# k2kobayashi/crank

Hardware: AMD Instinct MI355X
Metric: train frames/sec (higher is better)
Workload: dtype bf16

## Files before the change

### crank_amd/csrc/vq_kernels.hip

```cpp
#include "common.h"
#include "switches.h"
void conv_prof_begin(int cls, double flops, hipStream_t s);
void conv_prof_end(int cls, hipStream_t s);
void conv_prof_bytes(int cls, double bytes);

#define VQ_FRAMES 128
#define VQ_FIX_SCALE 268435456.0f
#define VQ_FIX_INV 3.7252902984619140625e-9f

template <int D>
__global__ __launch_bounds__(512) void vq_forward_kernel(const float* __restrict__ x, int ldx,
                                                         const float* __restrict__ cb, int N, int K, int kchunk,
                                                         long long* __restrict__ idx_out, float* __restrict__ e_out,
                                                         int lde, float* __restrict__ qx_out, int ldq) {
  extern __shared__ __attribute__((aligned(16))) unsigned char smem[];
  float* cbs = reinterpret_cast<float*>(smem);
  float* w2s = cbs + (size_t)kchunk * D;
  float* red_d = w2s + kchunk;
  int* red_i = reinterpret_cast<int*>(red_d + 4 * VQ_FRAMES);
  const int tid = threadIdx.x, lane = tid & 63, wave = tid >> 6;
  const int fg = wave & 1, cg = wave >> 1;
  const int fl = fg * 64 + lane;
  const long n = (long)blockIdx.x * VQ_FRAMES + fl;
  const bool valid = n < N;
// ... 365 lines not shown
    const long nw = (long)blockIdx.x * VQM_FB + fg * 32;
#pragma unroll
    for (int g = tp * (8 / TP); g < (tp + 1) * (8 / TP); g++) {
      const int f = 4 * g + sub;
      const int bi = __shfl(besti, f, 64);
      const long nf = nw + f;
      if (nf < N) {
        const float4 e = *reinterpret_cast<const float4*>(cb + (size_t)bi * D + c4);
        if (e_out) *reinterpret_cast<float4*>(e_out + nf * (long)lde + c4) = e;
        float4 xv = make_float4(0.f, 0.f, 0.f, 0.f);
        if (qx_out || fz.xsum || fz.cpart) {
          xv = *reinterpret_cast<const float4*>(x + nf * (long)ldx + c4);
          if (fz.add) {
            const float4 av = *reinterpret_cast<const float4*>(fz.add + nf * (long)fz.ldadd + c4);
            xv.x += av.x; xv.y += av.y; xv.z += av.z; xv.w += av.w;
          }
          if (fz.xsum) *reinterpret_cast<float4*>(fz.xsum + nf * (long)fz.ldsum + c4) = xv;
        }
        if (fz.cpart && (!fz.mask || fz.mask[nf])) {
          const float d0 = xv.x - e.x, d1 = xv.y - e.y, d2 = xv.z - e.z, d3 = xv.w - e.w;
          csum += d0 * d0; csum += d1 * d1; csum += d2 * d2; csum += d3 * d3;
          ccnt += 4.f;
        }
        if (qx_out) {
          float4 o;
          o.x = xv.x + (e.x - xv.x);
          o.y = xv.y + (e.y - xv.y);
          o.z = xv.z + (e.z - xv.z);
          o.w = xv.w + (e.w - xv.w);
          *reinterpret_cast<float4*>(qx_out + nf * (long)ldq + c4) = o;
        }
      }
    }
  }
  if (fz.cpart) {
#pragma unroll
    for (int o = 32; o > 0; o >>= 1) { csum += __shfl_xor(csum, o, 64); ccnt += __shfl_xor(ccnt, o, 64); }
    if (lane == 0) { vq_red[wave] = csum; vq_red[4 * TP + wave] = ccnt; }
    __syncthreads();
    if (tid == 0) {
      float a = vq_red[0], c = vq_red[4 * TP];
#pragma unroll
      for (int w = 1; w < 4 * TP; w++) { a += vq_red[w]; c += vq_red[4 * TP + w]; }
      fz.cpart[2 * blockIdx.x] = a; fz.cpart[2 * blockIdx.x + 1] = c;
    }
  }
  VQ_T(2)
}

typedef _Float16 vq_h8 __attribute__((ext_vector_type(8)));
typedef float vq_f32x2 __attribute__((ext_vector_type(2)));
typedef _Float16 vq_h4 __attribute__((ext_vector_type(4)));
#define VQH_KEY_EPS 1.6e-5f
#ifndef VQH_KEY_ABS
#define VQH_KEY_ABS 1.2e-38f
#endif
#define VQH_WS 68

__device__ unsigned long long vq_f16_flag_counts[3];
extern "C" int crk_debug_vq_flags(unsigned long long* host_out3, int reset) {
  if (hipMemcpyFromSymbol(host_out3, HIP_SYMBOL(vq_f16_flag_counts), 3 * sizeof(unsigned long long)) != hipSuccess) return 2;
  if (reset) {
    const unsigned long long z[3] = {0, 0, 0};
    if (hipMemcpyToSymbol(HIP_SYMBOL(vq_f16_flag_counts), z, sizeof(z)) != hipSuccess) return 2;
  }
  return 0;
}

__device__ __forceinline__ float vq_min_raw(float a, float b) {
  float r;
  asm("v_min_f32 %0, %1, %2" : "=v"(r) : "v"(a), "v"(b));
  return r;
}
struct VqTop3 { float m1, m2, m3; int i1, i2; };
__device__ __forceinline__ void vq_top3_insert(VqTop3& t, float v, int k) {
  const bool c1 = v < t.m1 || (v == t.m1 && k < t.i1);
  const bool c2 = v < t.m2 || (v == t.m2 && k < t.i2);
  t.m3 = c2 ? t.m2 : fminf(t.m3, v);
  t.i2 = c1 ? t.i1 : (c2 ? k : t.i2);
  t.m2 = c1 ? t.m1 : (c2 ? v : t.m2);
  t.i1 = c1 ? k : t.i1;
  t.m1 = c1 ? v : t.m1;
}
__device__ __forceinline__ void vq_top3_merge(VqTop3& t, float b1, float b2, float b3, int j1, int j2) {
  vq_top3_insert(t, b1, j1);
  vq_top3_insert(t, b2, j2);
  t.m3 = fminf(t.m3, b3);
}
__device__ __forceinline__ float vq_pow2(int e) { return __builtin_bit_cast(float, (unsigned)(e + 127) << 23); }
__device__ __forceinline__ int vq_expo(float v) { return (int)((__builtin_bit_cast(unsigned, v) >> 23) & 0xffu) - 127; }

#define VQ_PAD_W2 1.0e37f
__device__ __forceinline__ void vq_code_stats(const float* wrow, int k, int K, float& w2o, float& uswo, float& swso, float& wmxo) {
  float w2 = 0.f, am = 0.f;
#pragma unroll
  for (int q = 0; q < 16; q++) {
    const vq_f32x4 e = *reinterpret_cast<const vq_f32x4*>(wrow + 4 * q);
#pragma unroll
    for (int j = 0; j < 4; j++) { w2 = vq_sq_acc(w2, e[j]); am = fmaxf(am, fabsf(e[j])); }
  }
  w2o = k < K ? w2 : VQ_PAD_W2;
  const int er = 10 - vq_expo(am);
  const bool ok = am == 0.f || (w2 < INFINITY && er >= -60 && er <= 60);
  const int ewk = (ok && am > 0.f) ? er : 0;
  uswo = -2.f * vq_pow2(-ewk);
  swso = vq_pow2(ewk);
  wmxo = k < K ? (ok ? (w2 == w2 ? w2 : INFINITY) : INFINITY) : 0.f;
}
__device__ __forceinline__ void vq_plane_piece(vq_f32x4 pv, float sw, int k, int c, unsigned char* wh, unsigned char* wlo) {
  const int ct = k >> 5, i = k & 31, kc = c >> 2, h = (c & 3) >> 1;
  vq_h4 hi, lo;
#pragma unroll
  for (int jj = 0; jj < 4; jj++) {
    const float v = pv[jj] * sw;
    hi[jj] = (_Float16)v;
    lo[jj] = (_Float16)(v - (float)hi[jj]);
  }
  const size_t off = ((((size_t)ct * 4 + kc) * 64 + i + 32 * h) * 8 + 4 * (c & 1)) * 2;
  *reinterpret_cast<vq_h4*>(wh + off) = hi;
  *reinterpret_cast<vq_h4*>(wlo + off) = lo;
}
struct VqImgQ { const float* cb; unsigned char* img; int K; };
struct VqImgM { VqImgQ q[4]; };
__global__ __launch_bounds__(256) void vq_image_kernel(const VqImgM m) {
  __shared__ float wimg[32 * VQH_WS];
  __shared__ float sw_s[32];
  const VqImgQ e = m.q[blockIdx.y];
  const int K = e.K, KT = ((K + 63) >> 6) * 2, ct = blockIdx.x, tid = threadIdx.x;
  if (ct >= KT) return;
  vq_f32x4 pv[2];
#pragma unroll
  for (int j = 0; j < 2; j++) {
    const int pi = tid + 256 * j, k = ct * 32 + (pi >> 4);
    pv[j] = k < K ? *reinterpret_cast<const vq_f32x4*>(e.cb + (size_t)k * 64 + 4 * (pi & 15)) : vq_f32x4{0.f, 0.f, 0.f, 0.f};
    *reinterpret_cast<vq_f32x4*>(wimg + (size_t)(pi >> 4) * VQH_WS + 4 * (pi & 15)) = pv[j];
  }
  __syncthreads();
  float* tabs = reinterpret_cast<float*>(e.img + (size_t)KT * 8192);
  if (tid < 32) {
    const int k = ct * 32 + tid;
    float w2, us, sw, wm;
    vq_code_stats(wimg + (size_t)tid * VQH_WS, k, K, w2, us, sw, wm);
    tabs[k] = w2; tabs[KT * 32 + k] = us; tabs[2 * KT * 32 + k] = sw; tabs[3 * KT * 32 + k] = wm;
    sw_s[tid] = sw;
  }
  __syncthreads();
#pragma unroll
  for (int j = 0; j < 2; j++) {
    const int pi = tid + 256 * j;
    vq_plane_piece(pv[j], sw_s[pi >> 4], ct * 32 + (pi >> 4), pi & 15, e.img, e.img + (size_t)KT * 4096);
  }
}

template <int TP>
__global__ __launch_bounds__(256 * TP, 1) void vq_forward_f16_kernel(const float* __restrict__ x, int ldx,
                                                                     const float* __restrict__ cb, int N, int K,
                                                                     long long* __restrict__ idx_out, float* __restrict__ e_out,
                                                                     int lde, float* __restrict__ qx_out, int ldq, const VqFuse fz) {
  constexpr int D = 64, NT = 256 * TP;
  __shared__ float vq_red[8 * TP];
  __shared__ float vq_wmax[4 * TP];
  __shared__ float vq_m[TP][3][VQM_FB];
  __shared__ int vq_i[TP][2][VQM_FB];
  __shared__ float vq_xrow[4 * TP][D];
  extern __shared__ __attribute__((aligned(16))) unsigned char smem[];
  const int KT = ((K + 63) >> 6) * 2;
  unsigned char* wh = smem;
  unsigned char* wlo = smem + (size_t)KT * 4096;
  float* wimg = reinterpret_cast<float*>(smem);
  float* w2s = reinterpret_cast<float*>(smem + (size_t)KT * 32 * VQH_WS * 4);
  float* usw = w2s + KT * 32;
  float* sws = usw + KT * 32;
  const int tid = threadIdx.x, lane = tid & 63, l31 = lane & 31, half = lane >> 5;
  const int wave = __builtin_amdgcn_readfirstlane(tid >> 6), fg = wave & 3, tp = wave >> 2;
#ifdef VQ_PROF
  const unsigned long long vq_t0_ = __builtin_readcyclecounter();
#endif

  const long n = (long)blockIdx.x * VQM_FB + fg * 32 + l31;
  const bool valid = n < N;
  vq_f32x4 row[16];
  float w2max;
  if (fz.img) {
    constexpr int NPI = 16 / TP * 2;
    const vq_f32x4* src = reinterpret_cast<const vq_f32x4*>(fz.img);
    const float* tabs = reinterpret_cast<const float*>(fz.img + (size_t)KT * 8192);
    float* xt = reinterpret_cast<float*>(smem);
    constexpr int NXP = VQM_FB * 16 / NT;
    vq_f32x4 xv[NXP], av[NXP];
#pragma unroll
    for (int i = 0; i < NXP; i++) {
      const int pidx = tid + NT * i, f = pidx >> 4, c = pidx & 15;
      const long nf = (long)blockIdx.x * VQM_FB + f;
      xv[i] = nf < N ? *reinterpret_cast<const vq_f32x4*>(x + nf * (long)ldx + 4 * c) : vq_f32x4{0.f, 0.f, 0.f, 0.f};
      av[i] = (fz.add && nf < N) ? *reinterpret_cast<const vq_f32x4*>(fz.add + nf * (long)fz.ldadd + 4 * c) : vq_f32x4{0.f, 0.f, 0.f, 0.f};
    }
    vq_f32x4 pc[NPI];
#pragma unroll
    for (int j = 0; j < NPI; j++) { const int i = tid + NT * j; pc[j] = i < KT * 512 ? src[i] : vq_f32x4{0.f, 0.f, 0.f, 0.f}; }
    float tb[3];
#pragma unroll
    for (int j = 0; j < 3; j++) { const int i = tid + NT * j; tb[j] = i < 3 * KT * 32 ? tabs[i] : 0.f; }
    constexpr int NWM = (16 * 32 + NT - 1) / NT;
    float wm[NWM];
#pragma unroll
    for (int j = 0; j < NWM; j++) { const int k = tid + NT * j; wm[j] = k < KT * 32 ? tabs[3 * KT * 32 + k] : 0.f; }
#pragma unroll
    for (int i = 0; i < NXP; i++) {
      const int pidx = tid + NT * i;
      if (fz.add) xv[i] += av[i];
      if (fz.xsum_early) {
        const long nf = (long)blockIdx.x * VQM_FB + (pidx >> 4);
        if (nf < N) *reinterpret_cast<vq_f32x4*>(fz.xsum + nf * (long)fz.ldsum + 4 * (pidx & 15)) = xv[i];
      }
      *reinterpret_cast<vq_f32x4*>(xt + (size_t)(pidx >> 4) * VQH_WS + 4 * (pidx & 15)) = xv[i];
    }
    __syncthreads();
    {
      const float* xr = xt + (size_t)(fg * 32 + l31) * VQH_WS;
#pragma unroll
      for (int q = 0; q < 16; q++) row[q] = *reinterpret_cast<const vq_f32x4*>(xr + 4 * q);
    }
    __syncthreads();
    float wmx = 0.f;
#pragma unroll
    for (int j = 0; j < NWM; j++) wmx = fmaxf(wmx, wm[j]);
#pragma unroll
    for (int j = 0; j < NPI; j++) { const int i = tid + NT * j; if (i < KT * 512) reinterpret_cast<vq_f32x4*>(wh)[i] = pc[j]; }
#pragma unroll
    for (int j = 0; j < 3; j++) { const int i = tid + NT * j; if (i < 3 * KT * 32) w2s[i] = tb[j]; }
    for (int i = 3 * NT + tid; i < 3 * KT * 32; i += NT) w2s[i] = tabs[i];
#pragma unroll
    for (int o = 32; o > 0; o >>= 1) wmx = fmaxf(wmx, __shfl_xor(wmx, o, 64));
    if (lane == 0) vq_wmax[wave] = wmx;
    __syncthreads();
    w2max = vq_wmax[0];
#pragma unroll
    for (int w = 1; w < 4 * TP; w++) w2max = fmaxf(w2max, vq_wmax[w]);
  } else {
  {
    const float* xp = x + (valid ? n : 0) * (long)ldx;
#pragma unroll
    for (int q = 0; q < 16; q++) row[q] = *reinterpret_cast<const vq_f32x4*>(xp + 4 * q);
    if (fz.add) {
      const float* ap = fz.add + (valid ? n : 0) * (long)fz.ldadd;
#pragma unroll
      for (int q = 0; q < 16; q++) row[q] += *reinterpret_cast<const vq_f32x4*>(ap + 4 * q);
    }
  }
  constexpr int NPV = 16 / TP * 2;
  vq_f32x4 pv[NPV];
#pragma unroll
  for (int j = 0; j < NPV; j++) {
    const int pi = tid + NT * j, k = pi >> 4;
    pv[j] = (pi < KT * 32 * 16 && k < K) ? *reinterpret_cast<const vq_f32x4*>(cb + (size_t)pi * 4) : vq_f32x4{0.f, 0.f, 0.f, 0.f};
  }
#pragma unroll
  for (int j = 0; j < NPV; j++) {
    const int pi = tid + NT * j, k = pi >> 4, c = pi & 15;
    if (pi < KT * 32 * 16) *reinterpret_cast<vq_f32x4*>(wimg + (size_t)k * VQH_WS + 4 * c) = pv[j];
  }
  __syncthreads();
  float wmx = 0.f;
  for (int k = tid; k < KT * 32; k += NT) {
    float wm;
    vq_code_stats(wimg + (size_t)k * VQH_WS, k, K, w2s[k], usw[k], sws[k], wm);
    wmx = fmaxf(wmx, wm);
  }
#pragma unroll
  for (int o = 32; o > 0; o >>= 1) wmx = fmaxf(wmx, __shfl_xor(wmx, o, 64));
  if (lane == 0) vq_wmax[wave] = wmx;
  __syncthreads();
  w2max = vq_wmax[0];
#pragma unroll
  for (int w = 1; w < 4 * TP; w++) w2max = fmaxf(w2max, vq_wmax[w]);
  {
    float swk[NPV];
#pragma unroll
    for (int j = 0; j < NPV; j++) { const int pi = tid + NT * j; swk[j] = pi < KT * 32 * 16 ? sws[pi >> 4] : 1.f; }
#pragma unroll
    for (int j = 0; j < NPV; j++) {
      const int pi = tid + NT * j;
      if (pi < KT * 32 * 16) vq_plane_piece(pv[j], swk[j], pi >> 4, pi & 15, wh, wlo);
    }
  }
  }
  const bool w_ok = w2max < INFINITY;
  float x2 = 0.f, xmx = 0.f;
#pragma unroll
  for (int q = 0; q < 16; q++) {
#pragma unroll
    for (int j = 0; j < 4; j++) { x2 = vq_sq_acc(x2, row[q][j]); xmx = fmaxf(xmx, fabsf(row[q][j])); }
  }
  const int ex_raw = 10 - vq_expo(xmx);
  const bool x_ok = x2 < INFINITY && (xmx == 0.f || (ex_raw >= -60 && ex_raw <= 60));
  const int ex = (x_ok && xmx > 0.f) ? ex_raw : 0;
  vq_h8 xh[4], xl[4];
  {
    const float sx = vq_pow2(ex);
#pragma unroll
    for (int kc = 0; kc < 4; kc++)
#pragma unroll
      for (int j = 0; j < 8; j++) {
        const int d = 16 * kc + 8 * half + j;
        const float v0 = row[(16 * kc + j) >> 2][(16 * kc + j) & 3], v1 = row[(16 * kc + 8 + j) >> 2][(16 * kc + 8 + j) & 3];
        const float v = (half ? v1 : v0) * sx;
        (void)d;
        const _Float16 hi = (_Float16)v;
        xh[kc][j] = hi;
        xl[kc][j] = (_Float16)(v - (float)hi);
      }
  }
  const float sxinv = vq_pow2(-ex);
  __syncthreads();
  VQ_T(0)

  VqTop3 t;
  t.m1 = t.m2 = t.m3 = INFINITY;
  t.i1 = t.i2 = 0x7fffffff;
  const unsigned char* whl = wh + lane * 16;
  const unsigned char* wll = wlo + lane * 16;
#define VQH_TILE(aA, aB, ct, hc, lc, hn, ln)                                                                   \
  {                                                                                                            \
    _Pragma("unroll") for (int r = 0; r < 16; r++) { aA[r] = 0.f; aB[r] = 0.f; }                               \
    const size_t to_ = (size_t)((ct) + TP < KT ? (ct) + TP : (ct)) * 4096;                                     \
    _Pragma("unroll") for (int kc = 0; kc < 4; kc++) {                                                         \
      hn[kc] = *reinterpret_cast<const vq_h8*>(whl + to_ + kc * 1024);                                         \
      ln[kc] = *reinterpret_cast<const vq_h8*>(wll + to_ + kc * 1024);                                         \
    }                                                                                                          \
    _Pragma("unroll") for (int kc = 0; kc < 4; kc++) {                                                         \
      aA = __builtin_amdgcn_mfma_f32_32x32x16_f16(hc[kc], xh[kc], aA, 0, 0, 0);                                \
      aB = __builtin_amdgcn_mfma_f32_32x32x16_f16(lc[kc], xh[kc], aB, 0, 0, 0);                                \
      aB = __builtin_amdgcn_mfma_f32_32x32x16_f16(hc[kc], xl[kc], aB, 0, 0, 0);                                \
    }                                                                                                          \
  }
#define VQH_PICK(aA, aB, ct, tord) { const unsigned tagb_ = (unsigned)(tord) << 4; VQH_PICK_(aA, aB, ct) }
#define VQH_PICK_(aA, aB, ct)                                                                                  \
  _Pragma("unroll") for (int q = 0; q < 4; q++) {                                                              \
    const vq_f32x4 w2q = *reinterpret_cast<const vq_f32x4*>(w2s + (ct) * 32 + 8 * q + 4 * half);               \
    const vq_f32x4 usq = *reinterpret_cast<const vq_f32x4*>(usw + (ct) * 32 + 8 * q + 4 * half) * sxinv;       \
    _Pragma("unroll") for (int j2 = 0; j2 < 2; j2++) {                                                         \
      const vq_f32x2 acc = vq_f32x2{aA[4 * q + 2 * j2], aA[4 * q + 2 * j2 + 1]} +                              \
                           vq_f32x2{aB[4 * q + 2 * j2], aB[4 * q + 2 * j2 + 1]};                               \
      const vq_f32x2 v2 = __builtin_elementwise_fma(acc, vq_f32x2{usq[2 * j2], usq[2 * j2 + 1]},               \
                                                    vq_f32x2{w2q[2 * j2], w2q[2 * j2 + 1]});                   \
      const float vs_[2] = {v2.x, v2.y};      \
      _Pragma("unroll") for (int jj = 0; jj < 2; jj++) {                                                       \
        unsigned tag = tagb_ | (unsigned)(4 * q + 2 * j2 + jj);                                                \
        asm volatile("" : "+s"(tag));      \
        const float key = __builtin_bit_cast(float, (__builtin_bit_cast(unsigned, vs_[jj]) & keymask) | tag);  \
        t.m3 = __builtin_amdgcn_fmed3f(key, t.m2, t.m3);                                                       \
        t.m2 = __builtin_amdgcn_fmed3f(key, t.m1, t.m2);                                                       \
        t.m1 = vq_min_raw(key, t.m1);                                                                          \
      }                                                                                                        \
    }                                                                                                          \
  }
#define VQH_PAIR(nA, nB, ctn, hc, lc, hn, ln, pA, pB, ctp, tordp)                                              \
  VQH_TILE(nA, nB, ctn, hc, lc, hn, ln)                                                                        \
  VQH_PICK(pA, pB, ctp, tordp)                                                                                 \
  __builtin_amdgcn_sched_barrier(0);
  unsigned keymask = ~0x7fu;
  asm volatile("" : "+v"(keymask));
  f32x16 a0A, a0B, a1A, a1B;
  vq_h8 hA[4], lA[4], hB[4], lB[4];
#pragma unroll
  for (int kc = 0; kc < 4; kc++) {
    hA[kc] = *reinterpret_cast<const vq_h8*>(whl + (size_t)tp * 4096 + kc * 1024);
    lA[kc] = *reinterpret_cast<const vq_h8*>(wll + (size_t)tp * 4096 + kc * 1024);
  }
  VQH_TILE(a0A, a0B, tp, hA, lA, hB, lB)
  __builtin_amdgcn_sched_barrier(0);
  int tord = 0;
  for (int ct = tp; ct < KT - 2 * TP; ct += 2 * TP, tord += 2) {
    VQH_PAIR(a1A, a1B, ct + TP, hB, lB, hA, lA, a0A, a0B, ct, tord)
    VQH_PAIR(a0A, a0B, ct + 2 * TP, hA, lA, hB, lB, a1A, a1B, ct + TP, tord + 1)
  }
  VQH_PAIR(a1A, a1B, KT - TP + tp, hB, lB, hA, lA, a0A, a0B, KT - 2 * TP + tp, tord)
  VQH_PICK(a1A, a1B, KT - TP + tp, tord + 1)
#undef VQH_PAIR
#undef VQH_TILE
#undef VQH_PICK
  {
    const unsigned k1 = __builtin_bit_cast(unsigned, t.m1) & 0x7fu, k2 = __builtin_bit_cast(unsigned, t.m2) & 0x7fu;
    t.i1 = (int)((k1 >> 4) * TP + tp) * 32 + (int)(k1 & 3) + 8 * (int)((k1 >> 2) & 3) + 4 * half;
    t.i2 = (int)((k2 >> 4) * TP + tp) * 32 + (int)(k2 & 3) + 8 * (int)((k2 >> 2) & 3) + 4 * half;
  }
  {
    const float b1 = __shfl_xor(t.m1, 32, 64), b2 = __shfl_xor(t.m2, 32, 64), b3 = __shfl_xor(t.m3, 32, 64);
    const int j1 = __shfl_xor(t.i1, 32, 64), j2 = __shfl_xor(t.i2, 32, 64);
    vq_top3_merge(t, b1, b2, b3, j1, j2);
  }
  if (TP > 1) {
    if (half == 0) {
      const int f = fg * 32 + l31;
      vq_m[tp][0][f] = t.m1; vq_m[tp][1][f] = t.m2; vq_m[tp][2][f] = t.m3;
      vq_i[tp][0][f] = t.i1; vq_i[tp][1][f] = t.i2;
    }
    __syncthreads();
    const int f = fg * 32 + l31, o = tp ^ (TP - 1);
    vq_top3_merge(t, vq_m[o][0][f], vq_m[o][1][f], vq_m[o][2][f], vq_i[o][0][f], vq_i[o][1][f]);
  }
  VQ_T(3)
  const float xn = sqrtf(x2);
  const float w2a = w2s[(t.i1 >= 0 && t.i1 < KT * 32) ? t.i1 : 0];
  const float d1 = 2.0e-5f * xn * sqrtf(w2a) + 5.0e-7f * (x2 + w2a);
  const float p1 = VQH_KEY_EPS * fabsf(t.m1) + VQH_KEY_ABS;
  const float Rr = 2.001f * xn + sqrtf(fmaxf(t.m1 + p1 + d1, 0.f));
  const float wn = fminf(sqrtf(w2max), Rr * 1.001f);
  const float thr = d1 + 2.0e-5f * xn * wn + 5.0e-7f * (x2 + wn * wn);
  const bool trust = x_ok && w_ok && t.i1 < K;
  const bool sure = trust && (t.m2 - t.m1 > thr + p1 + (VQH_KEY_EPS * fabsf(t.m2) + VQH_KEY_ABS));
  const bool two = trust && !sure && (t.m3 - t.m1 > thr + p1 + (VQH_KEY_EPS * fabsf(t.m3) + VQH_KEY_ABS));
  const bool full = !sure && !two;
  int besti = t.i1;
  if (__builtin_amdgcn_ballot_w64(two)) {
    float dist = INFINITY;
    const int kc_ = half ? t.i2 : t.i1;
    if (two && kc_ < K) {
      const float* wp = cb + (size_t)kc_ * D;
      const float* xp = x + (valid ? n : 0) * (long)ldx;
      const float* ap = fz.add ? fz.add + (valid ? n : 0) * (long)fz.ldadd : nullptr;
      float dot = 0.f;
#pragma unroll
      for (int q = 0; q < 16; q++) {
        const vq_f32x4 wv = *reinterpret_cast<const vq_f32x4*>(wp + 4 * q);
        vq_f32x4 xv = *reinterpret_cast<const vq_f32x4*>(xp + 4 * q);
        if (ap) xv += *reinterpret_cast<const vq_f32x4*>(ap + 4 * q);
#pragma unroll
        for (int j = 0; j < 4; j++) dot = __builtin_fmaf(wv[j], xv[j], dot);
      }
      dist = (w2s[kc_] - 2.f * dot) + x2;
    }
    const float od = __shfl_xor(dist, 32, 64);
    const int oi = __shfl_xor(kc_, 32, 64);
    if (two) {
      const bool other = od < dist || (od == dist && oi < kc_);
      besti = other ? oi : kc_;
      if (!(dist < INFINITY) && !(od < INFINITY)) besti = 0x7fffffff;
    }
  }
  unsigned long long fm = __builtin_amdgcn_ballot_w64(full && half == 0);
  while (fm) {
    const int f = __builtin_ctzll(fm);
    fm &= fm - 1;
    {
      const long nf = (long)blockIdx.x * VQM_FB + fg * 32 + f;
      if (lane < 16) {
        vq_f32x4 xv = *reinterpret_cast<const vq_f32x4*>(x + (nf < N ? nf : 0) * (long)ldx + 4 * lane);
        if (fz.add) xv += *reinterpret_cast<const vq_f32x4*>(fz.add + (nf < N ? nf : 0) * (long)fz.ldadd + 4 * lane);
        *reinterpret_cast<vq_f32x4*>(&vq_xrow[wave][4 * lane]) = xv;
      }
      __builtin_amdgcn_fence(__ATOMIC_SEQ_CST, "wavefront");
    }
    const float fx2 = __shfl(x2, f, 64);
    float bd = INFINITY;
    int bi = 0x7fffffff;
    for (int k = lane; k < K; k += 64) {
      const float* wp = cb + (size_t)k * D;
      float dot = 0.f;
#pragma unroll
      for (int q = 0; q < 16; q++) {
        const vq_f32x4 wv = *reinterpret_cast<const vq_f32x4*>(wp + 4 * q);
        const vq_f32x4 xv = *reinterpret_cast<const vq_f32x4*>(&vq_xrow[wave][4 * q]);
#pragma unroll
        for (int j = 0; j < 4; j++) dot = __builtin_fmaf(wv[j], xv[j], dot);
      }
      const float dist = (w2s[k] - 2.f * dot) + fx2;
      if (dist < bd) { bd = dist; bi = k; }
    }
#pragma unroll
    for (int o = 32; o > 0; o >>= 1) {
      const float od = __shfl_xor(bd, o, 64);
      const int oi = __shfl_xor(bi, o, 64);
      if (od < bd || (od == bd && oi < bi)) { bd = od; bi = oi; }
    }
    if (l31 == f) besti = bi;
    __builtin_amdgcn_fence(__ATOMIC_SEQ_CST, "wavefront");
  }
  if (besti >= K) besti = 0;
  VQ_T(1)
  if (valid && half == 0 && tp == 0) {
    idx_out[n] = (long long)besti;
    if (!sure) atomicAdd(&vq_f16_flag_counts[two ? 1 : 2], 1ull);
  }
  float csum = 0.f, ccnt = 0.f;
  {
    constexpr int NG = 8 / TP;
    const int sub = lane >> 4, c4 = (lane & 15) * 4;
    const long nw = (long)blockIdx.x * VQM_FB + fg * 32;
    const bool want_x = qx_out || (fz.xsum && !fz.xsum_early) || fz.cpart;
    long nfs[NG];
    float4 ev[NG], xs[NG], as[NG];
    unsigned char mk[NG];
#pragma unroll
    for (int u = 0; u < NG; u++) {
      const int f = 4 * (tp * NG + u) + sub;
      const int bi = __shfl(besti, f, 64);
      nfs[u] = nw + f;
      const long nc = nfs[u] < N ? nfs[u] : 0;
      ev[u] = *reinterpret_cast<const float4*>(cb + (size_t)bi * D + c4);
      xs[u] = want_x ? *reinterpret_cast<const float4*>(x + nc * (long)ldx + c4) : make_float4(0.f, 0.f, 0.f, 0.f);
      as[u] = (want_x && fz.add) ? *reinterpret_cast<const float4*>(fz.add + nc * (long)fz.ldadd + c4) : make_float4(0.f, 0.f, 0.f, 0.f);
      mk[u] = (fz.cpart && fz.mask) ? fz.mask[nc] : (unsigned char)1;
    }
#pragma unroll
    for (int u = 0; u < NG; u++) {
      const long nf = nfs[u];
      if (nf < N) {
        const float4 e = ev[u];
        if (e_out) *reinterpret_cast<float4*>(e_out + nf * (long)lde + c4) = e;
        float4 xv = xs[u];
        if (want_x && fz.add) {
          xv.x += as[u].x; xv.y += as[u].y; xv.z += as[u].z; xv.w += as[u].w;
        }
        if (fz.xsum && !fz.xsum_early) *reinterpret_cast<float4*>(fz.xsum + nf * (long)fz.ldsum + c4) = xv;
        if (fz.cpart && mk[u]) {
          const float d0 = xv.x - e.x, d1 = xv.y - e.y, d2 = xv.z - e.z, d3 = xv.w - e.w;
          csum += d0 * d0; csum += d1 * d1; csum += d2 * d2; csum += d3 * d3;
          ccnt += 4.f;
        }
        if (qx_out) {
          float4 o;
          o.x = xv.x + (e.x - xv.x);
          o.y = xv.y + (e.y - xv.y);
          o.z = xv.z + (e.z - xv.z);
          o.w = xv.w + (e.w - xv.w);
          *reinterpret_cast<float4*>(qx_out + nf * (long)ldq + c4) = o;
        }
      }
    }
  }
  if (fz.cpart) {
#pragma unroll
    for (int o = 32; o > 0; o >>= 1) { csum += __shfl_xor(csum, o, 64); ccnt += __shfl_xor(ccnt, o, 64); }
    if (lane == 0) { vq_red[wave] = csum; vq_red[4 * TP + wave] = ccnt; }
    __syncthreads();
    if (tid == 0) {
      float a = vq_red[0], c = vq_red[4 * TP];
#pragma unroll
      for (int w = 1; w < 4 * TP; w++) { a += vq_red[w]; c += vq_red[4 * TP + w]; }
      fz.cpart[2 * blockIdx.x] = a; fz.cpart[2 * blockIdx.x + 1] = c;
    }
  }
  VQ_T(2)
}

static int vq_mfma_attrs() {
  static bool attr_set = false;
  if (!attr_set) {
    if (hipFuncSetAttribute((const void*)vq_forward_mfma_kernel<1>, hipFuncAttributeMaxDynamicSharedMemorySize, 160 * 1024 - 4096) != hipSuccess ||
        hipFuncSetAttribute((const void*)vq_forward_mfma_kernel<2>, hipFuncAttributeMaxDynamicSharedMemorySize, 160 * 1024 - 4096) != hipSuccess ||
        hipFuncSetAttribute((const void*)vq_forward_f16_kernel<2>, hipFuncAttributeMaxDynamicSharedMemorySize, 160 * 1024 - 12288) != hipSuccess)
      return CRK_ERR_HIP;
    attr_set = true;
  }
  return CRK_OK;
}
static int vq_f16_mode = -1;
extern "C" int crk_debug_vq_set_f16(int on) { vq_f16_mode = on ? 1 : 0; return 0; }
static bool vq_use_f16(int kt) {
  if (vq_f16_mode < 0) vq_f16_mode = crk_sw().vq_f16;
  return vq_f16_mode != 0 && kt % 4 == 0;
}
static void vq_mfma_launch(int nblk, int kt, size_t lds, hipStream_t s, const float* x, int ldx, const float* cb, int N, int K,
                           long long* idx, float* e, int lde, float* qx, int ldq, const VqFuse& fz) {
  const int tp_env = 2;
  conv_prof_bytes(7, 520.0 * N);
  conv_prof_begin(7, 2.0 * N * (double)K * 64.0, s);
  if (vq_use_f16(kt)) {
    const size_t lds16 = (size_t)kt * 32 * VQH_WS * 4 + (size_t)kt * 32 * 4 * 3;
    hipLaunchKernelGGL(vq_forward_f16_kernel<2>, dim3(nblk), dim3(512), lds16, s, x, ldx, cb, N, K, idx, e, lde, qx, ldq, fz);
    conv_prof_end(7, s);
    return;
  }
  if (tp_env == 2 && kt % 4 == 0)
    hipLaunchKernelGGL(vq_forward_mfma_kernel<2>, dim3(nblk), dim3(512), lds, s, x, ldx, cb, N, K, idx, e, lde, qx, ldq, fz);
  else
    hipLaunchKernelGGL(vq_forward_mfma_kernel<1>, dim3(nblk), dim3(256), lds, s, x, ldx, cb, N, K, idx, e, lde, qx, ldq, fz);
  conv_prof_end(7, s);
}

__global__ __launch_bounds__(256) void vq_commit_final_kernel(const float* __restrict__ part, int nblocks, float* __restrict__ out) {
  __shared__ float sh[8];
  float s = 0.f, c = 0.f;
  for (int i = threadIdx.x; i < nblocks; i += 256) { s += part[2 * i]; c += part[2 * i + 1]; }
#pragma unroll
  for (int o = 32; o > 0; o >>= 1) { s += __shfl_xor(s, o, 64); c += __shfl_xor(c, o, 64); }
  if ((threadIdx.x & 63) == 0) { sh[threadIdx.x >> 6] = s; sh[4 + (threadIdx.x >> 6)] = c; }
  __syncthreads();
  if (threadIdx.x == 0) {
    const float st = ((sh[0] + sh[1]) + sh[2]) + sh[3], ct = ((sh[4] + sh[5]) + sh[6]) + sh[7];
    out[0] = st / ct; out[1] = ct;
  }
}

extern "C" long long crk_vq_image_bytes(int K, int D) {
  if (D != 64 || K <= 0 || K > 512) return 0;
  const long long kt = ((K + 63) / 64) * 2;
  return kt * 8192 + kt * 32 * 4 * 4;
}
extern "C" int crk_vq_image_build_multi(int nq, const float* const* codebooks, const int* K, int D, void* const* images, void* stream) {
  if (nq < 1 || nq > 4 || !codebooks || !K || !images || D != 64) return CRK_ERR_ARG;
  VqImgM m;
  int ktmax = 0;
  for (int i = 0; i < nq; i++) {
    if (!codebooks[i] || !images[i] || K[i] <= 0 || K[i] > 512) return CRK_ERR_ARG;
    m.q[i].cb = codebooks[i]; m.q[i].img = (unsigned char*)images[i]; m.q[i].K = K[i];
    const int kt = ((K[i] + 63) / 64) * 2;
    if (kt > ktmax) ktmax = kt;
  }
  hipLaunchKernelGGL(vq_image_kernel, dim3(ktmax, nq), dim3(256), 0, (hipStream_t)stream, m);
  CRK_CHECK_LAUNCH();
  return CRK_OK;
}

extern "C" int crk_vq_forward_fused(const float* x, int ldx, const float* add, int ldadd, float* xsum, int ldsum,
                                    const float* codebook, int N, int D, int K, long long* idx, float* e, int lde, float* qx,
                                    int ldq, const unsigned char* mask, float* commit_out2, float* scratch, const void* image,
                                    void* stream) {
  if (!x || !codebook || !idx || N <= 0 || K <= 0) return CRK_ERR_ARG;
  if ((ldx & 3) || (lde & 3) || (ldq & 3) || (add && (ldadd & 3)) || (xsum && (ldsum & 3))) return CRK_ERR_ARG;
  if (commit_out2 && !scratch) return CRK_ERR_ARG;
  const int lc_env = crk_sw().vq_lc;
  const int nblk = (N + VQM_FB - 1) / VQM_FB;
  if (lc_env != 2 || D != 64 || K > 512 || nblk > 1024) return CRK_ERR_UNSUPPORTED;
  hipStream_t s = (hipStream_t)stream;
  if (vq_mfma_attrs() != CRK_OK) return CRK_ERR_HIP;
  const int kt = ((K + 63) / 64) * 2;
  const size_t lds = (size_t)kt * 32 * (D + 1) * 4;
  VqFuse fz; fz.add = add; fz.ldadd = ldadd; fz.xsum = xsum; fz.ldsum = ldsum; fz.mask = mask; fz.cpart = commit_out2 ? scratch : nullptr;
  fz.img = (const unsigned char*)image;
  {
    auto overlaps = [&](const float* p, int ld) {
      if (!p) return false;
      const char* a0 = (const char*)xsum; const char* a1 = a0 + (size_t)N * ldsum * 4;
      const char* b0 = (const char*)p; const char* b1 = b0 + (size_t)N * ld * 4;
      return a0 < b1 && b0 < a1;
    };
    fz.xsum_early = (fz.img && xsum && !overlaps(x, ldx) && !overlaps(add, ldadd)) ? 1 : 0;
  }
  vq_mfma_launch(nblk, kt, lds, s, x, ldx, codebook, N, K, idx, e, lde, qx, ldq, fz);
  if (commit_out2) hipLaunchKernelGGL(vq_commit_final_kernel, dim3(1), dim3(256), 0, s, scratch, nblk, commit_out2);
  CRK_CHECK_LAUNCH();
  return CRK_OK;
}

extern "C" int crk_vq_forward(const float* x, int ldx, const float* codebook, int N, int D, int K, long long* idx,
                              float* e, int lde, float* qx, int ldq, void* stream) {
  if (!x || !codebook || !idx || N <= 0 || K <= 0) return CRK_ERR_ARG;
  if ((ldx & 3) || (lde & 3) || (ldq & 3)) return CRK_ERR_ARG;
  hipStream_t s = (hipStream_t)stream;
  const int lc_env = crk_sw().vq_lc;
  if (lc_env == 2 && D == 64 && K <= 512) {
    if (vq_mfma_attrs() != CRK_OK) return CRK_ERR_HIP;
    const int kt = ((K + 63) / 64) * 2;
    const size_t lds = (size_t)kt * 32 * (D + 1) * 4;
    VqFuse fz{};
    vq_mfma_launch((N + VQM_FB - 1) / VQM_FB, kt, lds, s, x, ldx, codebook, N, K, idx, e, lde, qx, ldq, fz);
    CRK_CHECK_LAUNCH();
    return CRK_OK;
  }
  if (lc_env && D == 64 && K <= 512) {
    hipLaunchKernelGGL(vq_forward_lc_kernel<64>, dim3((N + VQL_FB - 1) / VQL_FB), dim3(512), 0, s, x, ldx, codebook, N, K, idx,
                       e, lde, qx, ldq);
    CRK_CHECK_LAUNCH();
    return CRK_OK;
  }
  int kchunk = K;
  const int max_floats = (150 * 1024 - 4 * VQ_FRAMES * 8) / 4;
  while ((size_t)kchunk * (D + 1) > (size_t)max_floats) kchunk = (kchunk + 1) / 2;
  const size_t lds = ((size_t)kchunk * (D + 1) + 4 * VQ_FRAMES * 2) * 4;
  dim3 grid((N + VQ_FRAMES - 1) / VQ_FRAMES), block(512);
#define VQ_LAUNCH(DD)                                                                                          \
  {                                                                                                            \
    static bool attr_set = false;                                                                              \
    if (!attr_set) {                                                                                           \
      if (hipFuncSetAttribute((const void*)vq_forward_kernel<DD>, hipFuncAttributeMaxDynamicSharedMemorySize,  \
                              160 * 1024) != hipSuccess) return CRK_ERR_HIP;                                   \
      attr_set = true;                                                                                         \
    }                                                                                                          \
    hipLaunchKernelGGL(vq_forward_kernel<DD>, grid, block, lds, s, x, ldx, codebook, N, K, kchunk, idx, e,     \
                       lde, qx, ldq);                                                                          \
  }
  if (D == 64) VQ_LAUNCH(64)
  else if (D == 32) VQ_LAUNCH(32)
  else if (D == 128) VQ_LAUNCH(128)
  else if (D == 16) VQ_LAUNCH(16)
  else return CRK_ERR_UNSUPPORTED;
#undef VQ_LAUNCH
  CRK_CHECK_LAUNCH();
  return CRK_OK;
}

__device__ __forceinline__ void vq_ema_partial_body(const float* __restrict__ x, int ldx, const long long* __restrict__ idx,
                                                    int N, int D, int K, int SW, int frames_per_chunk,
                                                    unsigned long long* __restrict__ part_sums, int* __restrict__ part_counts,
                                                    int chunk, int slice, unsigned char* vq_smem) {
  unsigned long long* acc = reinterpret_cast<unsigned long long*>(vq_smem);
  int* cnt = reinterpret_cast<int*>(acc + (size_t)SW * K);
  const int tid = threadIdx.x, d0 = slice * SW;
  const bool do_cnt = slice == 0;
  for (int i = tid; i < SW * K; i += 256) acc[i] = 0ull;
  if (do_cnt)
    for (int i = tid; i < K; i += 256) cnt[i] = 0;
  __syncthreads();
  const int qpf = SW >> 2, fpi = 256 / qpf;
  const int q = tid % qpf, fo = tid / qpf;
  const int n0 = chunk * frames_per_chunk, n1 = min(N, n0 + frames_per_chunk);
  const bool dok = d0 + 4 * q < D;
  for (int n = n0 + fo; n < n1; n += fpi) {
    const int k = (int)idx[n];
    if (dok) {
      const float4 f = *reinterpret_cast<const float4*>(x + (long)n * ldx + d0 + 4 * q);
      const float v[4] = {f.x, f.y, f.z, f.w};
#pragma unroll
      for (int j = 0; j < 4; j++)
        atomicAdd(acc + (size_t)(4 * q + j) * K + k, (unsigned long long)__float2ll_rn(v[j] * VQ_FIX_SCALE));
    }
    if (do_cnt && q == 0) atomicAdd(cnt + k, 1);
  }
  __syncthreads();
  const int sw = min(SW, D - d0);
  unsigned long long* dst = part_sums + ((size_t)chunk * D + d0) * K;
  for (int i = tid; i < sw * K; i += 256) dst[i] = acc[i];
// ... 496 lines not shown
```

Measured before the change: 21.62 million.

## Stream codebook image into LDS progressively, overlapping with MFMA distance tiles

Adds an IMG template parameter to the f16 VQ kernel. The precomputed codebook image is now loaded into registers per stage and written to LDS incrementally while early MFMA tiles run, so the kernel no longer waits for the full image before starting. Global loads are made unconditional by clamping the index, and the w2max reduction is deferred to after the main loop, which removes one barrier. The cost is more live registers, extra __syncthreads inside the early steps, and a more complex schedule that depends on nst.

```diff
diff --git a/crank_amd/csrc/vq_kernels.hip b/crank_amd/csrc/vq_kernels.hip
--- a/crank_amd/csrc/vq_kernels.hip
+++ b/crank_amd/csrc/vq_kernels.hip
@@ -541,7 +541,7 @@
   }
 }
 
-template <int TP>
+template <int TP, bool IMG>
 __global__ __launch_bounds__(256 * TP, 1) void vq_forward_f16_kernel(const float* __restrict__ x, int ldx,
                                                                      const float* __restrict__ cb, int N, int K,
                                                                      long long* __restrict__ idx_out, float* __restrict__ e_out,
@@ -569,39 +569,49 @@
   const long n = (long)blockIdx.x * VQM_FB + fg * 32 + l31;
   const bool valid = n < N;
   vq_f32x4 row[16];
-  float w2max;
-  if (fz.img) {
-    constexpr int NPI = 16 / TP * 2;
+  constexpr int NST = 16 / TP;
+  const int nst = KT / TP;
+  vq_f32x4* wh4 = reinterpret_cast<vq_f32x4*>(wh);
+  vq_f32x4 ph[NST], pl[NST];
+  if (IMG) {
     const vq_f32x4* src = reinterpret_cast<const vq_f32x4*>(fz.img);
     const float* tabs = reinterpret_cast<const float*>(fz.img + (size_t)KT * 8192);
     float* xt = reinterpret_cast<float*>(smem);
     constexpr int NXP = VQM_FB * 16 / NT;
+    const float* ap = fz.add ? fz.add : x;
+    const long lda = fz.add ? fz.ldadd : ldx;
     vq_f32x4 xv[NXP], av[NXP];
 #pragma unroll
     for (int i = 0; i < NXP; i++) {
       const int pidx = tid + NT * i, f = pidx >> 4, c = pidx & 15;
-      const long nf = (long)blockIdx.x * VQM_FB + f;
-      xv[i] = nf < N ? *reinterpret_cast<const vq_f32x4*>(x + nf * (long)ldx + 4 * c) : vq_f32x4{0.f, 0.f, 0.f, 0.f};
-      av[i] = (fz.add && nf < N) ? *reinterpret_cast<const vq_f32x4*>(fz.add + nf * (long)fz.ldadd + 4 * c) : vq_f32x4{0.f, 0.f, 0.f, 0.f};
-    }
-    vq_f32x4 pc[NPI];
-#pragma unroll
-    for (int j = 0; j < NPI; j++) { const int i = tid + NT * j; pc[j] = i < KT * 512 ? src[i] : vq_f32x4{0.f, 0.f, 0.f, 0.f}; }
-    float tb[3];
-#pragma unroll
-    for (int j = 0; j < 3; j++) { const int i = tid + NT * j; tb[j] = i < 3 * KT * 32 ? tabs[i] : 0.f; }
+      const long nf = (long)blockIdx.x * VQM_FB + f, nc = nf < N ? nf : N - 1;
+      xv[i] = *reinterpret_cast<const vq_f32x4*>(x + nc * (long)ldx + 4 * c);
+      av[i] = *reinterpret_cast<const vq_f32x4*>(ap + nc * lda + 4 * c);
+    }
+    __builtin_amdgcn_sched_barrier(0);
+    constexpr int NTB = (3 * 16 * 32 + NT - 1) / NT;
+    float tb[NTB];
+#pragma unroll
+    for (int j = 0; j < NTB; j++) { const int i = tid + NT * j; tb[j] = tabs[i < 3 * KT * 32 ? i : 3 * KT * 32 - 1]; }
     constexpr int NWM = (16 * 32 + NT - 1) / NT;
     float wm[NWM];
 #pragma unroll
-    for (int j = 0; j < NWM; j++) { const int k = tid + NT * j; wm[j] = k < KT * 32 ? tabs[3 * KT * 32 + k] : 0.f; }
+    for (int j = 0; j < NWM; j++) { const int k = tid + NT * j; wm[j] = tabs[3 * KT * 32 + (k < KT * 32 ? k : KT * 32 - 1)]; }
+    __builtin_amdgcn_sched_barrier(0);
+#pragma unroll
+    for (int st = 0; st < NST; st++) {
+      const int sl = st < nst ? st : 0;
+      ph[st] = src[sl * NT + tid];
+      pl[st] = src[KT * 256 + sl * NT + tid];
+      __builtin_amdgcn_sched_barrier(0);
+    }
 #pragma unroll
     for (int i = 0; i < NXP; i++) {
       const int pidx = tid + NT * i;
-      if (fz.add) xv[i] += av[i];
-      if (fz.xsum_early) {
-        const long nf = (long)blockIdx.x * VQM_FB + (pidx >> 4);
-        if (nf < N) *reinterpret_cast<vq_f32x4*>(fz.xsum + nf * (long)fz.ldsum + 4 * (pidx & 15)) = xv[i];
-      }
+      const long nf = (long)blockIdx.x * VQM_FB + (pidx >> 4);
+      xv[i] = fz.add ? xv[i] + av[i] : xv[i];
+      xv[i] = nf < N ? xv[i] : vq_f32x4{0.f, 0.f, 0.f, 0.f};
+      if (fz.xsum_early && nf < N) *reinterpret_cast<vq_f32x4*>(fz.xsum + nf * (long)fz.ldsum + 4 * (pidx & 15)) = xv[i];
       *reinterpret_cast<vq_f32x4*>(xt + (size_t)(pidx >> 4) * VQH_WS + 4 * (pidx & 15)) = xv[i];
     }
     __syncthreads();
@@ -611,21 +621,16 @@
       for (int q = 0; q < 16; q++) row[q] = *reinterpret_cast<const vq_f32x4*>(xr + 4 * q);
     }
     __syncthreads();
+#pragma unroll
+    for (int j = 0; j < NTB; j++) { const int i = tid + NT * j; if (i < 3 * KT * 32) w2s[i] = tb[j]; }
+    wh4[tid] = ph[0];
+    wh4[KT * 256 + tid] = pl[0];
     float wmx = 0.f;
 #pragma unroll
     for (int j = 0; j < NWM; j++) wmx = fmaxf(wmx, wm[j]);
-#pragma unroll
-    for (int j = 0; j < NPI; j++) { const int i = tid + NT * j; if (i < KT * 512) reinterpret_cast<vq_f32x4*>(wh)[i] = pc[j]; }
-#pragma unroll
-    for (int j = 0; j < 3; j++) { const int i = tid + NT * j; if (i < 3 * KT * 32) w2s[i] = tb[j]; }
-    for (int i = 3 * NT + tid; i < 3 * KT * 32; i += NT) w2s[i] = tabs[i];
 #pragma unroll
     for (int o = 32; o > 0; o >>= 1) wmx = fmaxf(wmx, __shfl_xor(wmx, o, 64));
     if (lane == 0) vq_wmax[wave] = wmx;
-    __syncthreads();
-    w2max = vq_wmax[0];
-#pragma unroll
-    for (int w = 1; w < 4 * TP; w++) w2max = fmaxf(w2max, vq_wmax[w]);
   } else {
   {
     const float* xp = x + (valid ? n : 0) * (long)ldx;
@@ -660,9 +665,6 @@
   for (int o = 32; o > 0; o >>= 1) wmx = fmaxf(wmx, __shfl_xor(wmx, o, 64));
   if (lane == 0) vq_wmax[wave] = wmx;
   __syncthreads();
-  w2max = vq_wmax[0];
-#pragma unroll
-  for (int w = 1; w < 4 * TP; w++) w2max = fmaxf(w2max, vq_wmax[w]);
   {
     float swk[NPV];
 #pragma unroll
@@ -674,7 +676,6 @@
     }
   }
   }
-  const bool w_ok = w2max < INFINITY;
   float x2 = 0.f, xmx = 0.f;
 #pragma unroll
   for (int q = 0; q < 16; q++) {
@@ -709,20 +710,6 @@
   t.i1 = t.i2 = 0x7fffffff;
   const unsigned char* whl = wh + lane * 16;
   const unsigned char* wll = wlo + lane * 16;
-#define VQH_TILE(aA, aB, ct, hc, lc, hn, ln)                                                                   \
-  {                                                                                                            \
-    _Pragma("unroll") for (int r = 0; r < 16; r++) { aA[r] = 0.f; aB[r] = 0.f; }                               \
-    const size_t to_ = (size_t)((ct) + TP < KT ? (ct) + TP : (ct)) * 4096;                                     \
-    _Pragma("unroll") for (int kc = 0; kc < 4; kc++) {                                                         \
-      hn[kc] = *reinterpret_cast<const vq_h8*>(whl + to_ + kc * 1024);                                         \
-      ln[kc] = *reinterpret_cast<const vq_h8*>(wll + to_ + kc * 1024);                                         \
-    }                                                                                                          \
-    _Pragma("unroll") for (int kc = 0; kc < 4; kc++) {                                                         \
-      aA = __builtin_amdgcn_mfma_f32_32x32x16_f16(hc[kc], xh[kc], aA, 0, 0, 0);                                \
-      aB = __builtin_amdgcn_mfma_f32_32x32x16_f16(lc[kc], xh[kc], aB, 0, 0, 0);                                \
-      aB = __builtin_amdgcn_mfma_f32_32x32x16_f16(hc[kc], xl[kc], aB, 0, 0, 0);                                \
-    }                                                                                                          \
-  }
 #define VQH_PICK(aA, aB, ct, tord) { const unsigned tagb_ = (unsigned)(tord) << 4; VQH_PICK_(aA, aB, ct) }
 #define VQH_PICK_(aA, aB, ct)                                                                                  \
   _Pragma("unroll") for (int q = 0; q < 4; q++) {                                                              \
@@ -744,10 +731,31 @@
       }                                                                                                        \
     }                                                                                                          \
   }
-#define VQH_PAIR(nA, nB, ctn, hc, lc, hn, ln, pA, pB, ctp, tordp)                                              \
-  VQH_TILE(nA, nB, ctn, hc, lc, hn, ln)                                                                        \
-  VQH_PICK(pA, pB, ctp, tordp)                                                                                 \
-  __builtin_amdgcn_sched_barrier(0);
+#define VQH_STEP(s, aA, aB, hc, lc, hn, ln, pA, pB)                                                          \
+  {                                                                                                            \
+    const size_t to_ = (size_t)(TP * ((s) + 1 < nst ? (s) + 1 : (s)) + tp) * 4096;                             \
+    _Pragma("unroll") for (int kc = 0; kc < 4; kc++) {                                                         \
+      hn[kc] = *reinterpret_cast<const vq_h8*>(whl + to_ + kc * 1024);                                         \
+      ln[kc] = *reinterpret_cast<const vq_h8*>(wll + to_ + kc * 1024);                                         \
+    }                                                                                                          \
+    _Pragma("unroll") for (int r = 0; r < 16; r++) { aA[r] = 0.f; aB[r] = 0.f; }                               \
+    _Pragma("unroll") for (int kc = 0; kc < 4; kc++) {                                                         \
+      aA = __builtin_amdgcn_mfma_f32_32x32x16_f16(hc[kc], xh[kc], aA, 0, 0, 0);                                \
+      aB = __builtin_amdgcn_mfma_f32_32x32x16_f16(lc[kc], xh[kc], aB, 0, 0, 0);                                \
+      aB = __builtin_amdgcn_mfma_f32_32x32x16_f16(hc[kc], xl[kc], aB, 0, 0, 0);                                \
+    }                                                                                                          \
+    if ((s) > 0) VQH_PICK(pA, pB, TP * ((s) - 1) + tp, (s) - 1)                                                \
+    __builtin_amdgcn_sched_barrier(0);                                                                         \
+    if (IMG && (s) < 2 && (s) + 2 < nst) {                                                                     \
+      _Pragma("unroll") for (int j_ = (s) + 2; j_ < ((s) == 0 ? 3 : NST); j_++) {                              \
+        if (j_ < nst) {                                                                                        \
+          wh4[j_ * NT + tid] = ph[j_];                                                                         \
+          wh4[KT * 256 + j_ * NT + tid] = pl[j_];                                                              \
+        }                                                                                                      \
+      }                                                                                                        \
+      __syncthreads();                                                                                         \
+    }                                                                                                          \
+  }
   unsigned keymask = ~0x7fu;
   asm volatile("" : "+v"(keymask));
   f32x16 a0A, a0B, a1A, a1B;
@@ -757,17 +765,19 @@
     hA[kc] = *reinterpret_cast<const vq_h8*>(whl + (size_t)tp * 4096 + kc * 1024);
     lA[kc] = *reinterpret_cast<const vq_h8*>(wll + (size_t)tp * 4096 + kc * 1024);
   }
-  VQH_TILE(a0A, a0B, tp, hA, lA, hB, lB)
-  __builtin_amdgcn_sched_barrier(0);
-  int tord = 0;
-  for (int ct = tp; ct < KT - 2 * TP; ct += 2 * TP, tord += 2) {
-    VQH_PAIR(a1A, a1B, ct + TP, hB, lB, hA, lA, a0A, a0B, ct, tord)
-    VQH_PAIR(a0A, a0B, ct + 2 * TP, hA, lA, hB, lB, a1A, a1B, ct + TP, tord + 1)
-  }
-  VQH_PAIR(a1A, a1B, KT - TP + tp, hB, lB, hA, lA, a0A, a0B, KT - 2 * TP + tp, tord)
-  VQH_PICK(a1A, a1B, KT - TP + tp, tord + 1)
-#undef VQH_PAIR
-#undef VQH_TILE
+  if (IMG) {
+    wh4[NT + tid] = ph[1];
+    wh4[KT * 256 + NT + tid] = pl[1];
+    __syncthreads();
+  }
+#pragma unroll
+  for (int st = 0; st < NST; st += 2) {
+    if (st >= nst) break;
+    VQH_STEP(st, a0A, a0B, hA, lA, hB, lB, a1A, a1B)
+    VQH_STEP(st + 1, a1A, a1B, hB, lB, hA, lA, a0A, a0B)
+  }
+  VQH_PICK(a1A, a1B, KT - TP + tp, nst - 1)
+#undef VQH_STEP
 #undef VQH_PICK
   {
     const unsigned k1 = __builtin_bit_cast(unsigned, t.m1) & 0x7fu, k2 = __builtin_bit_cast(unsigned, t.m2) & 0x7fu;
@@ -790,6 +800,10 @@
     vq_top3_merge(t, vq_m[o][0][f], vq_m[o][1][f], vq_m[o][2][f], vq_i[o][0][f], vq_i[o][1][f]);
   }
   VQ_T(3)
+  float w2max = vq_wmax[0];
+#pragma unroll
+  for (int w = 1; w < 4 * TP; w++) w2max = fmaxf(w2max, vq_wmax[w]);
+  const bool w_ok = w2max < INFINITY;
   const float xn = sqrtf(x2);
   const float w2a = w2s[(t.i1 >= 0 && t.i1 < KT * 32) ? t.i1 : 0];
   const float d1 = 2.0e-5f * xn * sqrtf(w2a) + 5.0e-7f * (x2 + w2a);
@@ -939,7 +953,8 @@
   if (!attr_set) {
     if (hipFuncSetAttribute((const void*)vq_forward_mfma_kernel<1>, hipFuncAttributeMaxDynamicSharedMemorySize, 160 * 1024 - 4096) != hipSuccess ||
         hipFuncSetAttribute((const void*)vq_forward_mfma_kernel<2>, hipFuncAttributeMaxDynamicSharedMemorySize, 160 * 1024 - 4096) != hipSuccess ||
-        hipFuncSetAttribute((const void*)vq_forward_f16_kernel<2>, hipFuncAttributeMaxDynamicSharedMemorySize, 160 * 1024 - 12288) != hipSuccess)
+        hipFuncSetAttribute((const void*)vq_forward_f16_kernel<2, false>, hipFuncAttributeMaxDynamicSharedMemorySize, 160 * 1024 - 12288) != hipSuccess ||
+        hipFuncSetAttribute((const void*)vq_forward_f16_kernel<2, true>, hipFuncAttributeMaxDynamicSharedMemorySize, 160 * 1024 - 12288) != hipSuccess)
       return CRK_ERR_HIP;
     attr_set = true;
   }
@@ -958,7 +973,10 @@
   conv_prof_begin(7, 2.0 * N * (double)K * 64.0, s);
   if (vq_use_f16(kt)) {
     const size_t lds16 = (size_t)kt * 32 * VQH_WS * 4 + (size_t)kt * 32 * 4 * 3;
-    hipLaunchKernelGGL(vq_forward_f16_kernel<2>, dim3(nblk), dim3(512), lds16, s, x, ldx, cb, N, K, idx, e, lde, qx, ldq, fz);
+    if (fz.img)
+      hipLaunchKernelGGL((vq_forward_f16_kernel<2, true>), dim3(nblk), dim3(512), lds16, s, x, ldx, cb, N, K, idx, e, lde, qx, ldq, fz);
+    else
+      hipLaunchKernelGGL((vq_forward_f16_kernel<2, false>), dim3(nblk), dim3(512), lds16, s, x, ldx, cb, N, K, idx, e, lde, qx, ldq, fz);
     conv_prof_end(7, s);
     return;
   }
```

Result: no change. 21.69 million (median of 6 runs) (+0.3%).
